# s-elkazdadi/ddp-pinocchio

Measured on AMD Instinct MI355X. Metric: DDP iterations/sec (fwd+bwd sweep), Talos nq=38 T=200, higher is better.
Workload: dtype f64

## Files before the change

ddp_pinocchio_amd/csrc/lin_static.hip:

```cpp
#include <float.h>
#include <math.h>
#include <stdlib.h>

#include <type_traits>
#include <utility>

#include "internal.h"
#include "lin_common.h"
#include "rbd.h"

#ifndef DEV_NO_EMIT
#define DEV_NO_EMIT 0
#endif
namespace {

struct TopoTalos38 {
  static constexpr int N = 38;
  static constexpr int parent[N] = {-1, 0, 1, 2, 3, 4,
                                    5, 6, 7, 8, 9, 10,
                                    5, 12, 13, 14, 15, 16,
                                    5, 18,
                                    19, 20, 21, 22, 23, 24, 25, 26,
                                    19, 28, 29, 30, 31, 32, 33, 34,
                                    19, 36};
  static constexpr int prismatic[N] = {1, 1, 1, 0, 0, 0, 0, 0, 0, 0, 0, 0, 0, 0, 0, 0, 0, 0, 0,
                                       0, 0, 0, 0, 0, 0, 0, 0, 0, 0, 0, 0, 0, 0, 0, 0, 0, 0, 0};
};

struct TopoChain6 {
  static constexpr int N = 6;
  static constexpr int parent[N] = {-1, 0, 1, 2, 3, 4};
  static constexpr int prismatic[N] = {0, 0, 0, 0, 0, 0};
};

}
#include "topo_extra.h"
namespace {

template <class T> constexpr bool has_child(int k) {
  for (int c = k + 1; c < T::N; ++c) if (T::parent[c] == k) return true;
  return false;
}
template <class T> constexpr int largest_child(int k) {
  int r = -1;
  for (int c = k + 1; c < T::N; ++c) if (T::parent[c] == k) r = c;
  return r;
}
template <class T> constexpr bool first_contrib(int k) { return T::parent[k] >= 0 && largest_child<T>(T::parent[k]) == k; }

template <class T>
bool topo_matches(const DevModel& m) {
  if (m.kind != DDP_HIP_MODEL_TREE || m.nv != T::N) return false;
  for (int i = 0; i < T::N; ++i)
    if (m.parent[i] != T::parent[i] || (m.jtype[i] == DDP_HIP_JOINT_PRISMATIC) != (T::prismatic[i] != 0)) return false;
  return true;
}

template <class T>
struct TauState {
  double acc[T::N][6];
  double uu[T::N];
};

template <class T, int K, int QS>
__device__ __forceinline__ void tau_up(const DevModel& m, const double* __restrict__ qc, const double* __restrict__ vc,
                                       double tauK, TauState<T>& s) {
  constexpr int o = T::prismatic[K] ? 3 : 0;
  const double* E = qc + K * QS;
  const double* r = E + 9;
  const double* U = E + 12;
  const double dinv = E[18];
  const double* pA0 = vc + K * rbd::VC_STRIDE + 6;
  const double* Iac = vc + K * rbd::VC_STRIDE + 12;
  const double* a = m.axis[K];
  double pAi[6];
  if constexpr (has_child<T>(K)) {
#pragma unroll
    for (int k = 0; k < 6; ++k) pAi[k] = s.acc[K][k];
  } else {
#pragma unroll
    for (int k = 0; k < 6; ++k) pAi[k] = pA0[k];
  }
  double sp = 0;
#pragma unroll
  for (int k = 0; k < 3; ++k) sp += a[k] * pAi[o + k];
  const double ui = tauK - sp;
  s.uu[K] = ui;
  constexpr int par = T::parent[K];
  if constexpr (par >= 0) {
    double pa[6], fp[6];
#pragma unroll
    for (int k = 0; k < 6; ++k) pa[k] = pAi[k] + Iac[k] + U[k] * (ui * dinv);
    rbd::xform_force_T(E, r, pa, fp);
    if constexpr (first_contrib<T>(K)) {
      const double* pp0 = vc + par * rbd::VC_STRIDE + 6;
#pragma unroll
      for (int k = 0; k < 6; ++k) s.acc[par][k] = pp0[k] + fp[k];
    } else {
#pragma unroll
      for (int k = 0; k < 6; ++k) s.acc[par][k] += fp[k];
    }
  }
  if constexpr (QS == rbd::QC_STRIDE || (K % 2) == 0) __builtin_amdgcn_sched_barrier(0);
}

template <class T, int K, int QS>
__device__ __forceinline__ void tau_down(const DevModel& m, const double* __restrict__ qc, const double* __restrict__ vc,
                                         TauState<T>& s) {
  constexpr int o = T::prismatic[K] ? 3 : 0;
  const double* E = qc + K * QS;
  const double* r = E + 9;
  const double* U = E + 12;
  const double dinv = E[18];
  const double* cb = vc + K * rbd::VC_STRIDE;
  double ap[6];
  constexpr int par = T::parent[K];
  if constexpr (par >= 0) rbd::xform_motion(E, r, s.acc[par], ap);
  else {
    const double a0[6] = {0, 0, 0, -m.gravity[0], -m.gravity[1], -m.gravity[2]};
    rbd::xform_motion(E, r, a0, ap);
  }
  double sum = 0;
#pragma unroll
  for (int k = 0; k < 6; ++k) { ap[k] += cb[k]; sum += U[k] * ap[k]; }
  const double qd = (s.uu[K] - sum) * dinv;
  s.uu[K] = qd;
  if constexpr (has_child<T>(K)) {
    const double* a = m.axis[K];
#pragma unroll
    for (int k = 0; k < 6; ++k) s.acc[K][k] = ap[k];
    s.acc[K][o] += a[0] * qd; s.acc[K][o + 1] += a[1] * qd; s.acc[K][o + 2] += a[2] * qd;
  }
  if constexpr (QS == rbd::QC_STRIDE || (K % 2) == 0) __builtin_amdgcn_sched_barrier(0);
}

template <class T, int QS, class TauFn, int... Ks>
__device__ __forceinline__ void tau_up_all(const DevModel& m, const double* __restrict__ qc, const double* __restrict__ vc, TauFn tau,
                                           TauState<T>& s, std::integer_sequence<int, Ks...>) {
  (tau_up<T, T::N - 1 - Ks, QS>(m, qc, vc, tau(T::N - 1 - Ks), s), ...);
}
template <class T, int QS, int HI, class TauFn, int... Ks>
__device__ __forceinline__ void tau_up_range(const DevModel& m, const double* __restrict__ qc, const double* __restrict__ vc, TauFn tau,
                                             TauState<T>& s, std::integer_sequence<int, Ks...>) {
  (tau_up<T, HI - Ks, QS>(m, qc, vc, tau(HI - Ks), s), ...);
}
template <class T, int QS, int... Ks>
__device__ __forceinline__ void tau_down_all(const DevModel& m, const double* __restrict__ qc, const double* __restrict__ vc,
                                             TauState<T>& s, std::integer_sequence<int, Ks...>) {
  (tau_down<T, Ks, QS>(m, qc, vc, s), ...);
}

constexpr int PS = 20;
template <int NV>
__device__ __forceinline__ void stage_placements(double* sp, const double* __restrict__ qc, int lane) {
  for (int idx = lane; idx < NV * 19; idx += LBS) {
    const int K = idx / 19, e = idx - K * 19;
    sp[K * PS + e] = qc[K * rbd::QC_STRIDE + e];
  }
}

template <class T> constexpr bool parents_at_least(int from, int lo) {
  for (int k = from; k < T::N; ++k) if (T::parent[k] < lo) return false;
  return true;
}
template <class T> constexpr int stage_split() {
  for (int kh = T::N / 2; kh > 0; --kh) if (parents_at_least<T>(kh + 1, kh)) return kh;
  return 0;
}

template <int NV, int K0, int K1, bool WITH_V = true>
struct StageRegs {
  static constexpr int NPW = (K1 - K0) * 19, NVW = WITH_V ? (K1 - K0) * rbd::VC_STRIDE : 0;
  static constexpr int CP = (NPW + LBS - 1) / LBS, CV = (NVW + LBS - 1) / LBS;
  double rp[CP], rv[CV > 0 ? CV : 1];
  __device__ __forceinline__ void load(const double* __restrict__ qc, const double* __restrict__ vc, int lane) {
#pragma unroll
    for (int c = 0; c < CP; ++c) {
      int idx = c * LBS + lane;
      idx = idx < NPW ? idx : NPW - 1;
      const int K = K0 + idx / 19, e = idx % 19;
      rp[c] = qc[K * rbd::QC_STRIDE + e];
    }
#pragma unroll
    for (int c = 0; c < CV; ++c) {
      int idx = c * LBS + lane;
      idx = idx < NVW ? idx : NVW - 1;
      rv[c] = vc[K0 * rbd::VC_STRIDE + idx];
    }
  }
  __device__ __forceinline__ void park(double* sp, double* sv, int lane) const {
#pragma unroll
    for (int c = 0; c < CP; ++c) {
      int idx = c * LBS + lane;
      idx = idx < NPW ? idx : NPW - 1;
      const int K = K0 + idx / 19, e = idx % 19;
      sp[K * PS + e] = rp[c];
    }
#pragma unroll
    for (int c = 0; c < CV; ++c) {
      int idx = c * LBS + lane;
      idx = idx < NVW ? idx : NVW - 1;
      sv[K0 * rbd::VC_STRIDE + idx] = rv[c];
    }
  }
};

__device__ __forceinline__ void tri_index(int64_t q, int Wd, int& ii, int& jj) {
  int a = (int)floor(((2.0 * Wd - 1.0) - sqrt((2.0 * Wd - 1.0) * (2.0 * Wd - 1.0) - 8.0 * (double)q)) * 0.5);
  if (a < 0) a = 0;
  while ((int64_t)a * (2 * Wd - a - 1) / 2 > q) --a;
  while ((int64_t)(a + 1) * (2 * Wd - a - 2) / 2 <= q) ++a;
  ii = a;
  jj = (int)(q - (int64_t)a * (2 * Wd - a - 1) / 2) + a + 1;
}

template <int NV, int NP = LBS>
struct OutStage {
  double qdd[NP * (NV + 1)];
  int pij[NP];
};

template <int NV, int NP>
__device__ __forceinline__ void offdiag_emit(const LinParams& p, OutStage<NV, NP>& S, bool valid, int i, int j, int64_t bt,
                                             const double* __restrict__ xg, double dt, int pass = 0) {
  constexpr int n = 2 * NV, mm = NV;
  constexpr int RW = 16, NJ = (n + RW - 1) / RW, GRP = LBS / RW, PPG = NP / GRP, NB = NP == LBS ? 2 : 1;
  static_assert(PPG % NB == 0, "points per group");
  const double eps = sqrt(sqrt(DBL_EPSILON));
  const double eps2 = eps * eps;
  const int lane = threadIdx.x;
  if (lane / NP == pass) S.pij[lane % NP] = i | (j << 8) | ((valid ? 1 : 0) << 16);
  double* const fxx = p.fxx + bt * n * n * n;
  double* const fux = p.fux + bt * n * mm * n;
  double* const fuu = p.fuu + bt * n * mm * mm;
  const double* const fxb = p.fx + bt * n * n;
  const double* const fub = p.fu + bt * n * mm;
  __syncthreads();
  const int kk = lane % RW, grp = lane / RW;
  const double* f0 = p.f_val + bt * n;
  double f0k[NJ], xk[NJ], xvk[NJ];
#pragma unroll
  for (int jx = 0; jx < NJ; ++jx) {
    const int k = kk + RW * jx;
    const int kc = k < n ? k : n - 1;
    f0k[jx] = f0[kc];
    xk[jx] = xg[kc];
    xvk[jx] = kc < NV ? xg[NV + kc] : 0.0;
  }
  if (DEV_NO_EMIT) return;
  for (int pt = 0; pt < PPG; pt += NB) {
    double a1[NB][NJ], a2[NB][NJ], d1[NB][NJ], d2[NB][NJ];
    double* o0[NB];
    double* o1[NB];
    int ie[NB], je[NB], ee[NB];
#pragma unroll
    for (int u = 0; u < NB; ++u) {
      const int e = (pt + u) * GRP + grp;
      ee[u] = e;
      const int pk = S.pij[e];
      const int i1 = pk & 255, j1 = (pk >> 8) & 255;
      ie[u] = i1;
      je[u] = j1;
      const bool at_x_1 = i1 < n, at_x_2 = j1 < n;
      const int idx_1 = at_x_1 ? i1 : i1 - n, idx_2 = at_x_2 ? j1 : j1 - n;
      double* tensor;
      int L;
      if (at_x_1) { if (at_x_2) { tensor = fxx; L = n; } else { tensor = fux; L = mm; } }
      else { tensor = fuu; L = mm; }
      o0[u] = (pk >> 16) ? tensor + (int64_t)idx_2 * n + (int64_t)idx_1 * n * L : nullptr;
      o1[u] = ((pk >> 16) && at_x_1 == at_x_2 && !p.skip_qv_mirror) ? tensor + (int64_t)idx_1 * n + (int64_t)idx_2 * n * L : nullptr;
      if (o0[u]) {
        const double* q0 = at_x_1 ? fxb + (int64_t)idx_1 * n : fub + (int64_t)idx_1 * n;
        const double* q1 = at_x_2 ? fxb + (int64_t)idx_2 * n : fub + (int64_t)idx_2 * n;
        const double* q2 = at_x_1 ? fxx + (int64_t)idx_1 * n + (int64_t)idx_1 * n * n : fuu + (int64_t)idx_1 * n + (int64_t)idx_1 * n * mm;
        const double* q3 = at_x_2 ? fxx + (int64_t)idx_2 * n + (int64_t)idx_2 * n * n : fuu + (int64_t)idx_2 * n + (int64_t)idx_2 * n * mm;
#pragma unroll
        for (int jx = 0; jx < NJ; ++jx) {
          const int k = kk + RW * jx;
          const int kc = k < n ? k : n - 1;
          a1[u][jx] = q0[kc]; a2[u][jx] = q1[kc]; d1[u][jx] = q2[kc]; d2[u][jx] = q3[kc];
        }
      }
    }
#pragma unroll
    for (int u = 0; u < NB; ++u) {
      if (!o0[u]) continue;
#pragma unroll
      for (int jx = 0; jx < NJ; ++jx) {
        const int k = kk + RW * jx;
        if (k >= n) continue;
        if (p.skip_top && k < NV && !((ie[u] < n && ie[u] % NV == k) || (je[u] < n && je[u] % NV == k))) continue;
        double xs = k == ie[u] ? xk[jx] + eps : xk[jx];
        if (k == je[u]) xs = xs + eps;
        double fv;
        if (k < NV) {
          double xv = (NV + k) == ie[u] ? xvk[jx] + eps : xvk[jx];
          if (NV + k == je[u]) xv = xv + eps;
          const double vo = dt * xv;
          fv = xs + vo;
        } else {
          fv = xs + S.qdd[ee[u] * (NV + 1) + (k - NV)] * dt;
        }
        double df = fv - f0k[jx];
        df -= eps * a1[u][jx];
        df -= eps * a2[u][jx];
        df *= 2;
        const double val = 0.5 * (df / eps2 - d1[u][jx] - d2[u][jx]);
        o0[u][k] = val;
        if (o1[u]) o1[u][k] = val;
      }
    }
  }
}

template <int NV>
struct RowStage {
  double q[(NV + 2) * (NV + 1)];
};

template <int NV, bool DIAG_ROW, class ST>
__device__ __forceinline__ void rowblock_emit(const ST& S, int lane, int i, int jb, double* __restrict__ out, double* __restrict__ mirror,
                                              int64_t mstride, const double* __restrict__ a2, const double* __restrict__ d2, int64_t dstride,
                                              double dt, const double* __restrict__ f0g, const double* __restrict__ a1g,
                                              double* __restrict__ d1g, const double* __restrict__ xg, bool skip_top = false) {
  constexpr int n = 2 * NV, RW = 16, NJ = (n + RW - 1) / RW, CG = LBS / RW, NIT = (NV + CG - 1) / CG;
  const int r1 = i % NV;
  const double eps = sqrt(sqrt(DBL_EPSILON));
  const double eps2 = eps * eps;
  const int kk = lane % RW, cg = lane / RW;
  double xk[NJ], xvk[NJ], f0k[NJ], a1k[NJ], d1k[NJ];
#pragma unroll
  for (int j = 0; j < NJ; ++j) {
    const int k = kk + RW * j;
    const int kc = k < n ? k : n - 1;
    f0k[j] = f0g[kc];
    a1k[j] = a1g[kc];
    double x = xg[kc];
    if (kc == i) x = x + eps;
    xk[j] = x;
    double xv = xg[kc < NV ? NV + kc : kc];
    if (NV + kc == i) xv = xv + eps;
    xvk[j] = xv;
    if constexpr (DIAG_ROW) {
      double fv;
      if (kc < NV) {
        const double vo = dt * xv;
        fv = x + vo;
      } else {
        fv = x + S.q[NV * (NV + 1) + (kc - NV)] * dt;
      }
      double df = fv - f0k[j];
      df -= eps * a1k[j];
      df *= 2;
      const double dd = df / eps2;
      d1k[j] = dd;
      if (cg == 0 && k < n && !(skip_top && k < NV && k != r1)) d1g[k] = dd;
    } else {
      d1k[j] = d1g[kc];
    }
  }
  double va2[2][NJ], vd2[2][NJ];
  auto fetch = [&](int it, double (&A)[NJ], double (&D)[NJ]) {
    const int c = it * CG + cg;
    const int cc = c < NV ? c : NV - 1;
#pragma unroll
    for (int j = 0; j < NJ; ++j) {
      const int k = kk + RW * j;
      const int kc = k < n ? k : n - 1;
      A[j] = a2[kc + cc * n];
      D[j] = d2[kc + cc * dstride];
    }
  };
  auto form = [&](int it, const double (&A)[NJ], const double (&D)[NJ]) {
    const int c = it * CG + cg;
    const bool cv = c < NV;
    const int cc = cv ? c : NV - 1;
    const int jp = jb + cc;
#pragma unroll
    for (int j = 0; j < NJ; ++j) {
      const int k = kk + RW * j;
      if (!(cv && k < n)) continue;
      if (skip_top && k < NV && k != r1 && !(jp < n && jp % NV == k)) continue;
      double x = xk[j];
      if (k == jp) x = x + eps;
      double fv;
      if (k < NV) {
        double xv = xvk[j];
        if (NV + k == jp) xv = xv + eps;
        const double vo = dt * xv;
        fv = x + vo;
      } else {
        fv = x + S.q[cc * (NV + 1) + (k - NV)] * dt;
      }
      double df = fv - f0k[j];
      df -= eps * a1k[j];
      df -= eps * A[j];
      df *= 2;
      const double val = 0.5 * (df / eps2 - d1k[j] - D[j]);
      out[k + c * n] = val;
      if (mirror) mirror[k + c * mstride] = val;
    }
  };
  if (DEV_NO_EMIT) return;
  fetch(0, va2[0], vd2[0]);
  for (int it = 0; it < NIT; it += 2) {
    if (it + 1 < NIT) fetch(it + 1, va2[1], vd2[1]);
    form(it, va2[0], vd2[0]);
    if (it + 1 < NIT) {
      if (it + 2 < NIT) fetch(it + 2, va2[0], vd2[0]);
      form(it + 1, va2[1], vd2[1]);
    }
  }
}

template <class T, bool ROWS>
__global__ __launch_bounds__(LBS, ROWS ? 1 : 3) void lin_static_tau_kernel(LinParams p) {
  constexpr int nv = T::N, n = 2 * nv;
  constexpr int TRI = nv * (nv - 1) / 2, GU = (TRI + LBS - 1) / LBS, G = ROWS ? 2 * nv : GU;
  const int64_t bt = blockIdx.x / G;
  const int g = (int)(blockIdx.x % G) + (ROWS ? 0 : 2 * nv);
  const int lane = threadIdx.x;
  const int64_t Tn = p.d.T;
  const int b = (int)(bt / Tn);
  const int64_t t = bt % Tn;
  const DevModel& m = *p.model;
  int i, j, cfg, vcfg;
  bool valid;
  if (g < nv) { i = g; j = n + lane; cfg = 1 + g; vcfg = nv + 1 + g; valid = lane < nv; }
  else if (g < 2 * nv) { i = g; j = n + lane; cfg = 0; vcfg = 1 + (g - nv); valid = lane < nv; }
  else {
    const int pid = (g - 2 * nv) * LBS + lane;
    valid = pid < TRI;
    tri_index(valid ? pid : 0, nv, i, j);
    i += n; j += n; cfg = 0; vcfg = 0;
  }
  const double eps = sqrt(sqrt(DBL_EPSILON));
  const double* __restrict__ qc = p.qcache + (bt * (nv + 1) + cfg) * (int64_t)nv * rbd::QC_STRIDE;
  const double* __restrict__ vc = p.vcache + (bt * (2 * nv + 1) + vcfg) * (int64_t)nv * rbd::VC_STRIDE;
  const double* __restrict__ xg = p.x + ((int64_t)b * (Tn + 1) + t) * n;
  const double* __restrict__ ug = p.u + ((int64_t)b * Tn + t) * nv;
  const int iu = i - n, ju = j - n;
  __shared__ union TauLds { double P[nv * PS + nv * rbd::VC_STRIDE]; RowStage<nv> S; OutStage<nv, LBS / 2> O; } s_lds;
  double* s_P = s_lds.P;
  double* s_V = s_P + nv * PS;
  constexpr int KH = stage_split<T>();
  StageRegs<nv, 0, (KH > 0) ? KH : 1> lower;
  {
    StageRegs<nv, KH, nv> upper;
    upper.load(qc, vc, lane);
    lower.load(qc, vc, lane);
    upper.park(s_P, s_V, lane);
    rbd::coop_sync<true>();
  }
  TauState<T> s;
  auto tau = [&](int k) { double v = ug[k]; if (k == iu) v = v + eps; if (k == ju) v = v + eps; return v; };
  static_assert(parents_at_least<T>(KH + 1, KH), "the first half of the pass must not reach below record KH");
  tau_up_range<T, PS, nv - 1>(m, s_P, s_V, tau, s, std::make_integer_sequence<int, nv - 1 - KH>{});
  lower.park(s_P, s_V, lane);
  rbd::coop_sync<true>();
  tau_up_range<T, PS, KH>(m, s_P, s_V, tau, s, std::make_integer_sequence<int, KH + 1>{});
  tau_down_all<T, PS>(m, s_P, s_V, s, std::make_integer_sequence<int, nv>{});
  __builtin_amdgcn_sched_barrier(0);
  typedef __attribute__((address_space(4))) const LinParams* kernarg_t;
  const kernarg_t kp = (kernarg_t)__builtin_amdgcn_kernarg_segment_ptr();
  if constexpr (ROWS) {
    RowStage<nv>& S = s_lds.S;
    const int mm = nv;
    __syncthreads();
    const int row = lane <= nv ? lane : nv + 1;
#pragma unroll
    for (int k = 0; k < nv; ++k) S.q[row * (nv + 1) + k] = s.uu[k];
    __syncthreads();
    rowblock_emit<nv, true>(S, lane, i, n, kp->fux + bt * n * mm * n + (int64_t)i * n * mm, nullptr, 0, kp->fu + bt * n * mm,
                            kp->fuu + bt * n * mm * mm, (int64_t)n + (int64_t)n * mm, m.dt, kp->f_val + bt * n,
                            kp->fx + bt * n * n + (int64_t)i * n, kp->fxx + bt * n * n * n + (int64_t)i * n + (int64_t)i * n * n, xg, kp->skip_top != 0);
  } else {
    OutStage<nv, LBS / 2>& S = s_lds.O;
    LinParams po;
    po.f_val = kp->f_val; po.fx = kp->fx; po.fu = kp->fu; po.fxx = kp->fxx; po.fux = kp->fux; po.fuu = kp->fuu; po.skip_qv_mirror = kp->skip_qv_mirror; po.skip_top = kp->skip_top;
    const double dt = m.dt;
    __syncthreads();
#pragma unroll 1
    for (int pass = 0; pass < 2; ++pass) {
      if (pass) __syncthreads();
      if (lane / (LBS / 2) == pass) {
#pragma unroll
        for (int k = 0; k < nv; ++k) S.qdd[(lane % (LBS / 2)) * (nv + 1) + k] = s.uu[k];
      }
      offdiag_emit<nv, LBS / 2>(po, S, valid, i, j, bt, xg, dt, pass);
    }
  }
}

template <class T> constexpr int n_children(int k) {
  int c = 0;
  for (int j = k + 1; j < T::N; ++j) if (T::parent[j] == k) ++c;
  return c;
}
template <class T> constexpr bool chain_start(int k) { return T::parent[k] < 0 || T::parent[k] != k - 1 || n_children<T>(T::parent[k]) > 1; }
template <class T> constexpr bool chain_end(int k) { return k == T::N - 1 || chain_start<T>(k + 1); }
template <class T> constexpr int chain_first(int k) { while (!chain_start<T>(k)) --k; return k; }
template <class T> constexpr int max_chain() {
  int best = 1;
  for (int k = 0; k < T::N; ++k)
    if (chain_end<T>(k)) { const int len = k - chain_first<T>(k) + 1; if (len > best) best = len; }
  return best;
}

template <class T>
struct VelState {
  double vel[T::N][6];
  double acc[T::N][6];
  double uu[T::N];
};

template <int UQS_, int QS_ = rbd::QC_STRIDE>
struct VelCtx {
  static constexpr int UQS = UQS_;
  static constexpr int QS = QS_;
  const DevModel* m;
  const double* qp;
  const double* __restrict__ qc;
  const double* __restrict__ xg;
  const double* __restrict__ ug;
  double* uq;
  int i, j;
  double eps;
  template <int K> __device__ __forceinline__ const double* er(double*) const { return qp + K * QS; }
  template <int K> __device__ __forceinline__ const double* er_down(double* b) const { return er<K>(b); }
  template <int K> __device__ __forceinline__ const double* ud() const { return qp + K * QS + 12; }
  template <int K> __device__ __forceinline__ void ia_cb(const double*, const double* cb, double* Iac) const { rbd::sym6_mv(qc + K * rbd::QC_STRIDE + 19, cb, Iac); }
  template <int K> __device__ __forceinline__ const double* ud_down() const { return ud<K>(); }
};

template <int NV, class C>
__device__ __forceinline__ double lane_v(const C& c, int K) {
  double v = c.xg[NV + K];
  if (NV + K == c.i) v = v + c.eps;
  if (NV + K == c.j) v = v + c.eps;
  return v;
}

template <class T, int K, class C>
__device__ __forceinline__ void joint_vel(const C& c, const double* vel_par, double* vel) {
  constexpr int o = T::prismatic[K] ? 3 : 0;
  double Pb[12];
  const double* E = c.template er<K>(Pb);
  const double* r = E + 9;
  const double* a = c.m->axis[K];
  const double vK = lane_v<T::N>(c, K);
  double vJ[6] = {0, 0, 0, 0, 0, 0};
  vJ[o] = a[0] * vK; vJ[o + 1] = a[1] * vK; vJ[o + 2] = a[2] * vK;
  if constexpr (T::parent[K] >= 0) rbd::xform_motion(E, r, vel_par, vel);
  else {
#pragma unroll
    for (int k = 0; k < 6; ++k) vel[k] = 0.0;
  }
#pragma unroll
  for (int k = 0; k < 6; ++k) vel[k] += vJ[k];
}
template <class T, int K, class C>
__device__ __forceinline__ void vel_from_root(const C& c, double* vel) {
  if constexpr (T::parent[K] >= 0) {
    double vp[6];
    vel_from_root<T, T::parent[K]>(c, vp);
    joint_vel<T, K>(c, vp, vel);
  } else {
    joint_vel<T, K>(c, nullptr, vel);
  }
}
template <class T, int K, class C>
__device__ __forceinline__ void bias_force0(const C& c, const double* vel, double* pA) {
  double Iv[6];
  rbd::sym6_mv(c.m->I6[K], vel, Iv);
  rbd::crf(vel, Iv, pA);
}

template <class T, int K, int E, class C>
__device__ __forceinline__ void chain_down(const C& c, VelState<T>& s) {
  if constexpr (T::parent[K] >= 0) joint_vel<T, K>(c, s.vel[T::parent[K]], s.vel[K]);
  else joint_vel<T, K>(c, nullptr, s.vel[K]);
  __builtin_amdgcn_sched_barrier(0);
  if constexpr (K < E) chain_down<T, K + 1, E>(c, s);
}

template <class T, int K, int F, class C>
__device__ __forceinline__ void chain_up(const C& c, VelState<T>& s) {
  constexpr int o = T::prismatic[K] ? 3 : 0;
  double Pb[12];
  const double* E = c.template er<K>(Pb);
  const double* r = E + 9;
  const double* U = c.template ud<K>();
  const double dinv = U[6];
  const double* a = c.m->axis[K];
  double pAi[6];
  if constexpr (has_child<T>(K)) {
#pragma unroll
    for (int k = 0; k < 6; ++k) pAi[k] = s.acc[K][k];
  } else {
    bias_force0<T, K>(c, s.vel[K], pAi);
  }
  double sp = 0;
#pragma unroll
  for (int k = 0; k < 3; ++k) sp += a[k] * pAi[o + k];
  const double ui = c.ug[K] - sp;
  if constexpr (C::UQS == 0) s.uu[K] = ui; else c.uq[K * C::UQS] = ui;
  constexpr int par = T::parent[K];
  if constexpr (par >= 0) {
    const double vK = lane_v<T::N>(c, K);
    double vJ[6] = {0, 0, 0, 0, 0, 0}, cb[6], pa[6], Iac[6], fp[6];
    vJ[o] = a[0] * vK; vJ[o + 1] = a[1] * vK; vJ[o + 2] = a[2] * vK;
    rbd::crm(s.vel[K], vJ, cb);
    c.template ia_cb<K>(U, cb, Iac);
#pragma unroll
    for (int k = 0; k < 6; ++k) pa[k] = pAi[k] + Iac[k] + U[k] * (ui * dinv);
    rbd::xform_force_T(E, r, pa, fp);
    if constexpr (first_contrib<T>(K)) {
      double p0[6];
      bias_force0<T, par>(c, s.vel[par], p0);
#pragma unroll
      for (int k = 0; k < 6; ++k) s.acc[par][k] = p0[k] + fp[k];
    } else {
#pragma unroll
      for (int k = 0; k < 6; ++k) s.acc[par][k] += fp[k];
    }
  }
  __builtin_amdgcn_sched_barrier(0);
  if constexpr (K > F) chain_up<T, K - 1, F>(c, s);
}

template <class T, int K, class C>
__device__ __forceinline__ void chain_at(const C& c, VelState<T>& s) {
  if constexpr (chain_end<T>(K)) {
    constexpr int F = chain_first<T>(K), P = T::parent[F];
    if constexpr (P >= 0) {
      if constexpr (first_contrib<T>(F) && n_children<T>(P) > 1) vel_from_root<T, P>(c, s.vel[P]);
    }
    chain_down<T, F, K>(c, s);
    chain_up<T, K, F>(c, s);
  }
}
template <class T, class C, int... Ks>
__device__ __forceinline__ void vel_up_all(const C& c, VelState<T>& s, std::integer_sequence<int, Ks...>) {
  (chain_at<T, T::N - 1 - Ks>(c, s), ...);
}

template <class T, int K, class C>
__device__ __forceinline__ void vel_down(const C& c, VelState<T>& s) {
  constexpr int o = T::prismatic[K] ? 3 : 0;
  constexpr int par = T::parent[K];
  double Pb[12];
  const double* E = c.template er_down<K>(Pb);
  const double* r = E + 9;
  const double* U = c.template ud_down<K>();
  const double dinv = U[6];
  const double* a = c.m->axis[K];
  const double vK = lane_v<T::N>(c, K);
  double vJ[6] = {0, 0, 0, 0, 0, 0}, vel[6], cb[6], ap[6];
  vJ[o] = a[0] * vK; vJ[o + 1] = a[1] * vK; vJ[o + 2] = a[2] * vK;
  if constexpr (par >= 0) {
    rbd::xform_motion(E, r, s.vel[par], vel);
    rbd::xform_motion(E, r, s.acc[par], ap);
  } else {
    const double a0[6] = {0, 0, 0, -c.m->gravity[0], -c.m->gravity[1], -c.m->gravity[2]};
#pragma unroll
    for (int k = 0; k < 6; ++k) vel[k] = 0.0;
    rbd::xform_motion(E, r, a0, ap);
  }
#pragma unroll
  for (int k = 0; k < 6; ++k) vel[k] += vJ[k];
  rbd::crm(vel, vJ, cb);
  double sum = 0;
#pragma unroll
  for (int k = 0; k < 6; ++k) { ap[k] += cb[k]; sum += U[k] * ap[k]; }
  double ui;
  if constexpr (C::UQS == 0) ui = s.uu[K]; else ui = c.uq[K * C::UQS];
  const double qd = (ui - sum) * dinv;
  if constexpr (C::UQS == 0) s.uu[K] = qd; else c.uq[K * C::UQS] = qd;
  if constexpr (has_child<T>(K)) {
#pragma unroll
    for (int k = 0; k < 6; ++k) { s.vel[K][k] = vel[k]; s.acc[K][k] = ap[k]; }
    s.acc[K][o] += a[0] * qd; s.acc[K][o + 1] += a[1] * qd; s.acc[K][o + 2] += a[2] * qd;
  }
  __builtin_amdgcn_sched_barrier(0);
}
template <class T, class C, int... Ks>
__device__ __forceinline__ void vel_down_all(const C& c, VelState<T>& s, std::integer_sequence<int, Ks...>) {
  (vel_down<T, Ks>(c, s), ...);
}

template <class T, bool ROWS>
__global__ __launch_bounds__(LBS, ROWS ? 3 : 2) void lin_static_vel_kernel(LinParams p) {
  constexpr int nv = T::N, n = 2 * nv;
  constexpr int TRI = nv * (nv - 1) / 2, GU = (TRI + LBS - 1) / LBS, G = ROWS ? nv : GU;
  const int64_t bt = blockIdx.x / G;
  const int g = (int)(blockIdx.x % G);
  const int lane = threadIdx.x;
  const int64_t Tn = p.d.T;
  const int b = (int)(bt / Tn);
  const int64_t t = bt % Tn;
  int i, j, cfg;
  bool valid;
  if (ROWS) { i = g; j = nv + lane; cfg = 1 + g; valid = lane < nv; }
  else {
    const int pid = g * LBS + lane;
    valid = pid < TRI;
    tri_index(valid ? pid : 0, nv, i, j);
    i += nv; j += nv; cfg = 0;
  }
  struct PairStage { OutStage<nv, LBS / 2> O; double spare[nv + 1]; };
  using Stage = typename std::conditional<ROWS, RowStage<nv>, PairStage>::type;
  __shared__ union VelLds { Stage S; double P[nv * rbd::QC_STRIDE]; } s_lds;
  Stage& S = s_lds.S;
  double* s_P = s_lds.P;
  VelCtx<0, rbd::QC_STRIDE> c;
  c.m = p.model;
  c.qc = p.qcache + (bt * (nv + 1) + cfg) * (int64_t)nv * rbd::QC_STRIDE;
  c.qp = s_P;
  c.xg = p.x + ((int64_t)b * (Tn + 1) + t) * n;
  c.ug = p.u + ((int64_t)b * Tn + t) * nv;
  c.i = i; c.j = j;
  c.eps = sqrt(sqrt(DBL_EPSILON));
  c.uq = nullptr;
  {
    constexpr int NW = nv * rbd::QC_STRIDE, CW = (NW + LBS - 1) / LBS;
    double rq[CW];
#pragma unroll
    for (int r = 0; r < CW; ++r) { const int idx = r * LBS + lane; rq[r] = c.qc[idx < NW ? idx : NW - 1]; }
#pragma unroll
    for (int r = 0; r < CW; ++r) { const int idx = r * LBS + lane; s_P[idx < NW ? idx : NW - 1] = rq[r]; }
    c.qc = s_P;
    rbd::coop_sync<true>();
  }
  VelState<T> s;
  vel_up_all<T>(c, s, std::make_integer_sequence<int, nv>{});
  vel_down_all<T>(c, s, std::make_integer_sequence<int, nv>{});
  __builtin_amdgcn_sched_barrier(0);
  typedef __attribute__((address_space(4))) const LinParams* kernarg_t;
  const kernarg_t kp = (kernarg_t)__builtin_amdgcn_kernarg_segment_ptr();
  const double dt = c.m->dt;
  if constexpr (ROWS) {
    double* fxx = kp->fxx + bt * n * n * n;
    const double* fxb = kp->fx + bt * n * n;
    __syncthreads();
    const int row = valid ? lane : nv;
#pragma unroll
    for (int k = 0; k < nv; ++k) S.q[row * (nv + 1) + k] = s.uu[k];
    __syncthreads();
    rowblock_emit<nv, false>(S, lane, i, nv, fxx + (int64_t)nv * n + (int64_t)i * n * n,
                             kp->skip_qv_mirror ? nullptr : fxx + (int64_t)i * n + (int64_t)nv * n * n, (int64_t)n * n,
                             fxb + (int64_t)nv * n, fxx + (int64_t)nv * n + (int64_t)nv * n * n, (int64_t)n + (int64_t)n * n, dt,
                             kp->f_val + bt * n, fxb + (int64_t)i * n, fxx + (int64_t)i * n + (int64_t)i * n * n, c.xg, kp->skip_top != 0);
  } else {
    constexpr int NP = LBS / 2;
    LinParams po;
    po.f_val = kp->f_val; po.fx = kp->fx; po.fu = kp->fu; po.fxx = kp->fxx; po.fux = kp->fux; po.fuu = kp->fuu; po.skip_qv_mirror = kp->skip_qv_mirror; po.skip_top = kp->skip_top;
    __syncthreads();
    double* const own = &S.O.qdd[(lane % NP) * (nv + 1)];
    double* const row = lane < NP ? own : S.spare;
#pragma unroll
    for (int k = 0; k < nv; ++k) row[k] = s.uu[k];
#pragma unroll 1
    for (int pass = 0; pass < 2; ++pass) {
      if (pass) {
        __syncthreads();
        if (lane >= NP) {
#pragma unroll
          for (int k = 0; k < nv; ++k) own[k] = s.uu[k];
        }
      }
      offdiag_emit<nv, NP>(po, S.O, valid, i, j, bt, c.xg, dt, pass);
    }
  }
}

constexpr int WS_PER_JOINT = 8;

template <class T>
// ... 593 lines not shown
  if constexpr (!DIAG) {
    if (double* ao = kp->accel_out) {
      ao += bt * (3 * nv + 1) * nv;
      double* al = ao + (LEVEL - 1) * nv * nv;
      for (int e = lane; e < nv * nv; e += LBS) { const int c = e / nv; al[e] = s_q[c * (nv + 1) + (e - c * nv)]; }
      if (LEVEL == 2 && lane < nv) ao[3 * nv * nv + lane] = s_q[nv * (nv + 1) + lane];
      return;
    }
  }
  double* fcol = LEVEL == 3 ? kp->fu + bt * n * nv : kp->fx + bt * n * n + (LEVEL == 2 ? nv * n : 0);
  double* out = fcol;
  int64_t ostride = n;
  if constexpr (DIAG) {
    if (LEVEL == 3) { out = kp->fuu + bt * n * nv * nv; ostride = n + (int64_t)n * nv; }
    else { ostride = n + (int64_t)n * n; out = kp->fxx + bt * n * n * n + (LEVEL == 2 ? nv * ostride : 0); }
  }
  first_output<nv, DIAG>(s_q, lane, LEVEL == 1 ? 0 : (LEVEL == 2 ? nv : n), out, ostride, fcol, kp->f_val + bt * n, xg, model->dt, eps, kp->skip_top != 0);
}

template <class T, int K>
__device__ __forceinline__ void placement_static(const DevModel& m, double q, double* P) {
  const double* Rp = m.Rp[K];
  const double* a = m.axis[K];
  double* E = P;
  double* r = P + 9;
  if constexpr (!T::prismatic[K]) {
    double sn, cs;
    sincos(q, &sn, &cs);
    const double Kx[9] = {0, -a[2], a[1], a[2], 0, -a[0], -a[1], a[0], 0};
    double K2[9], RJ[9], Rc[9];
    rbd::mm3(Kx, Kx, K2);
    const double omc = 1.0 - cs;
#pragma unroll
    for (int k = 0; k < 9; ++k) RJ[k] = sn * Kx[k] + omc * K2[k];
    RJ[0] += 1.0; RJ[4] += 1.0; RJ[8] += 1.0;
    rbd::mm3(Rp, RJ, Rc);
#pragma unroll
    for (int k = 0; k < 3; ++k)
#pragma unroll
      for (int l = 0; l < 3; ++l) E[3 * k + l] = Rc[3 * l + k];
    r[0] = m.pp[K][0]; r[1] = m.pp[K][1]; r[2] = m.pp[K][2];
  } else {
    const double dd[3] = {a[0] * q, a[1] * q, a[2] * q};
    double Rd[3];
    rbd::mv3(Rp, dd, Rd);
#pragma unroll
    for (int k = 0; k < 3; ++k)
#pragma unroll
      for (int l = 0; l < 3; ++l) E[3 * k + l] = Rp[3 * l + k];
    r[0] = m.pp[K][0] + Rd[0]; r[1] = m.pp[K][1] + Rd[1]; r[2] = m.pp[K][2] + Rd[2];
  }
}

struct QvCtx {
  const DevModel* __restrict__ m;
  const double* __restrict__ xg;
  double* __restrict__ qc;
  double* __restrict__ vc;
  double* lvel;
  int jn;
  double eps;
};
template <class T>
struct QvState {
  double vel[T::N][6];
  double accI[T::N][21];
};
template <class T, int K>
__device__ __forceinline__ void qv_placement(const QvCtx& c, double* P) {
  double q = c.xg[K];
  if (K == c.jn) q = q + c.eps;
  placement_static<T, K>(*c.m, q, P);
}
template <class T, int K>
__device__ __forceinline__ void qv_joint_vel(const QvCtx& c, const double* P, const double* vel_par, double* vel) {
  constexpr int o = T::prismatic[K] ? 3 : 0;
  const double* a = c.m->axis[K];
  const double vK = c.xg[T::N + K];
  double vJ[6] = {0, 0, 0, 0, 0, 0};
  vJ[o] = a[0] * vK; vJ[o + 1] = a[1] * vK; vJ[o + 2] = a[2] * vK;
  if constexpr (T::parent[K] >= 0) rbd::xform_motion(P, P + 9, vel_par, vel);
  else {
#pragma unroll
    for (int k = 0; k < 6; ++k) vel[k] = 0.0;
  }
#pragma unroll
  for (int k = 0; k < 6; ++k) vel[k] += vJ[k];
}
template <class T, int K>
__device__ __forceinline__ void qv_vel_from_root(const QvCtx& c, double* vel) {
  double P[12];
  qv_placement<T, K>(c, P);
  if constexpr (T::parent[K] >= 0) {
    double vp[6];
    qv_vel_from_root<T, T::parent[K]>(c, vp);
    qv_joint_vel<T, K>(c, P, vp, vel);
  } else {
    qv_joint_vel<T, K>(c, P, nullptr, vel);
  }
}
template <class T, int K, int F, int E>
__device__ __forceinline__ void qv_chain_down(const QvCtx& c, double* cur) {
  double P[12], vel[6];
  qv_placement<T, K>(c, P);
  if constexpr (T::parent[K] >= 0) qv_joint_vel<T, K>(c, P, cur, vel);
  else qv_joint_vel<T, K>(c, P, nullptr, vel);
#pragma unroll
  for (int k = 0; k < 6; ++k) { cur[k] = vel[k]; c.lvel[((K - F) * 6 + k) * LBS] = vel[k]; }
  __builtin_amdgcn_sched_barrier(0);
  if constexpr (K < E) qv_chain_down<T, K + 1, F, E>(c, cur);
}
template <class T, int K, int F>
__device__ __forceinline__ void qv_chain_up(const QvCtx& c, QvState<T>& s) {
  constexpr int o = T::prismatic[K] ? 3 : 0;
  const double* a = c.m->axis[K];
  double P[12], IA[21], U[6], Ia[21], vel[6];
  qv_placement<T, K>(c, P);
#pragma unroll
  for (int k = 0; k < 6; ++k) vel[k] = c.lvel[((K - F) * 6 + k) * LBS];
  if constexpr (has_child<T>(K)) {
#pragma unroll
    for (int k = 0; k < 21; ++k) IA[k] = s.accI[K][k];
  } else {
#pragma unroll
    for (int k = 0; k < 21; ++k) IA[k] = c.m->I6[K][k];
  }
  double d = 0;
#pragma unroll
  for (int r = 0; r < 6; ++r) U[r] = IA[rbd::sidx(r, o)] * a[0] + IA[rbd::sidx(r, o + 1)] * a[1] + IA[rbd::sidx(r, o + 2)] * a[2];
#pragma unroll
  for (int k = 0; k < 3; ++k) d += a[k] * U[o + k];
  const double dinv = 1.0 / d;
#pragma unroll
  for (int r = 0; r < 6; ++r)
#pragma unroll
    for (int cc = 0; cc <= r; ++cc) Ia[rbd::sidx(r, cc)] = IA[rbd::sidx(r, cc)] - U[r] * U[cc] * dinv;
  constexpr int par = T::parent[K];
  if constexpr (par >= 0) {
    if constexpr (first_contrib<T>(K)) {
#pragma unroll
      for (int k = 0; k < 21; ++k) s.accI[par][k] = c.m->I6[par][k];
    }
    rbd::add_xtix(P, P + 9, Ia, s.accI[par]);
  }
  const double vK = c.xg[T::N + K];
  double vJ[6] = {0, 0, 0, 0, 0, 0}, cb[6], pA[6], Iv[6], Iac[6];
  vJ[o] = a[0] * vK; vJ[o + 1] = a[1] * vK; vJ[o + 2] = a[2] * vK;
  rbd::crm(vel, vJ, cb);
  rbd::sym6_mv(c.m->I6[K], vel, Iv);
  rbd::crf(vel, Iv, pA);
  rbd::sym6_mv(Ia, cb, Iac);
  double* qo = c.qc + K * rbd::QC_STRIDE;
#pragma unroll
  for (int k = 0; k < 12; ++k) qo[k] = P[k];
#pragma unroll
  for (int k = 0; k < 6; ++k) qo[12 + k] = U[k];
  qo[18] = dinv;
#pragma unroll
  for (int k = 0; k < 21; ++k) qo[19 + k] = Ia[k];
  double* vo = c.vc + K * rbd::VC_STRIDE;
#pragma unroll
  for (int k = 0; k < 6; ++k) { vo[k] = cb[k]; vo[6 + k] = pA[k]; vo[12 + k] = Iac[k]; }
  __builtin_amdgcn_sched_barrier(0);
  if constexpr (K > F) qv_chain_up<T, K - 1, F>(c, s);
}
template <class T, int K>
__device__ __forceinline__ void qv_chain_at(const QvCtx& c, QvState<T>& s) {
  if constexpr (chain_end<T>(K)) {
    constexpr int F = chain_first<T>(K), P = T::parent[F];
    double cur[6] = {0, 0, 0, 0, 0, 0};
    if constexpr (P >= 0) {
      if constexpr (first_contrib<T>(F) && n_children<T>(P) > 1) qv_vel_from_root<T, P>(c, s.vel[P]);
#pragma unroll
      for (int k = 0; k < 6; ++k) cur[k] = s.vel[P][k];
    }
    qv_chain_down<T, F, F, K>(c, cur);
    qv_chain_up<T, K, F>(c, s);
  }
}
template <class T, int... Ks>
__device__ __forceinline__ void qv_all(const QvCtx& c, QvState<T>& s, std::integer_sequence<int, Ks...>) {
  (qv_chain_at<T, T::N - 1 - Ks>(c, s), ...);
}

template <class T>
__global__ __launch_bounds__(LBS, 2) void lin_static_qvcache_kernel(LinParams p, const DevModel* __restrict__ model, const double* __restrict__ xs,
                                                                 double* __restrict__ qcache, double* __restrict__ vcache) {
  constexpr int nv = T::N, n = 2 * nv, MAXCH = max_chain<T>();
  const int lane = threadIdx.x;
  const int64_t Tn = p.d.T;
  const int64_t e = (int64_t)blockIdx.x * LBS + lane;
  const int64_t bt = e / p.ncfg;
  const int cfgi = (int)(e - bt * p.ncfg);
  const int b = (int)(bt / Tn);
  const int64_t t = bt % Tn;
  __shared__ double s_vel[MAXCH * 6 * LBS];
  if (bt >= p.d.batch * Tn) return;
  QvCtx c;
  c.m = model;
  c.xg = xs + ((int64_t)b * (Tn + 1) + t) * n;
  c.qc = qcache + (bt * p.ncfg + cfgi) * (int64_t)nv * rbd::QC_STRIDE;
  c.vc = vcache + (bt * p.nvcfg + (cfgi == 0 ? 0 : nv + cfgi)) * (int64_t)nv * rbd::VC_STRIDE;
  c.lvel = s_vel + lane;
  c.jn = cfgi - 1;
  c.eps = sqrt(sqrt(DBL_EPSILON));
  QvState<T> s;
  qv_all<T>(c, s, std::make_integer_sequence<int, nv>{});
}

template <class T, int K>
__device__ __forceinline__ void vc_joint(const DevModel& m, const double* __restrict__ qc, const double* __restrict__ xg, int iv, double eps,
                                         double (&vel)[T::N][6], double* __restrict__ vc) {
  constexpr int o = T::prismatic[K] ? 3 : 0;
  const double* E = qc + K * rbd::QC_STRIDE;
  const double* r = E + 9;
  const double* Ia = E + 19;
  const double* a = m.axis[K];
  double vK = xg[T::N + K];
  if (K == iv) vK = vK + eps;
  double vJ[6] = {0, 0, 0, 0, 0, 0}, v[6], cb[6], pA[6], Iv[6], Iac[6];
  vJ[o] = a[0] * vK; vJ[o + 1] = a[1] * vK; vJ[o + 2] = a[2] * vK;
  if constexpr (T::parent[K] >= 0) rbd::xform_motion(E, r, vel[T::parent[K]], v);
  else {
#pragma unroll
    for (int k = 0; k < 6; ++k) v[k] = 0.0;
  }
#pragma unroll
  for (int k = 0; k < 6; ++k) { v[k] += vJ[k]; vel[K][k] = v[k]; }
  rbd::crm(v, vJ, cb);
  rbd::sym6_mv(m.I6[K], v, Iv);
  rbd::crf(v, Iv, pA);
  rbd::sym6_mv(Ia, cb, Iac);
  double* vo = vc + K * rbd::VC_STRIDE;
#pragma unroll
  for (int k = 0; k < 6; ++k) { vo[k] = cb[k]; vo[6 + k] = pA[k]; vo[12 + k] = Iac[k]; }
  __builtin_amdgcn_sched_barrier(0);
}
template <class T, int... Ks>
__device__ __forceinline__ void vc_all(const DevModel& m, const double* __restrict__ qc, const double* __restrict__ xg, int iv, double eps,
                                       double (&vel)[T::N][6], double* __restrict__ vc, std::integer_sequence<int, Ks...>) {
  (vc_joint<T, Ks>(m, qc, xg, iv, eps, vel, vc), ...);
}
template <class T>
__global__ __launch_bounds__(LBS) void lin_static_vcache_kernel(LinParams p, const DevModel* __restrict__ model, const double* __restrict__ xs,
                                                                const double* __restrict__ qcache, double* __restrict__ vcache) {
  constexpr int nv = T::N, n = 2 * nv;
  const int64_t bt = blockIdx.x;
  const int lane = threadIdx.x;
  const int64_t Tn = p.d.T;
  const int b = (int)(bt / Tn);
  const int64_t t = bt % Tn;
  if (lane >= nv) return;
  const double* __restrict__ qc = qcache + (bt * (nv + 1)) * (int64_t)nv * rbd::QC_STRIDE;
  const double* __restrict__ xg = xs + ((int64_t)b * (Tn + 1) + t) * n;
  double* __restrict__ vc = vcache + (bt * (2 * nv + 1) + 1 + lane) * (int64_t)nv * rbd::VC_STRIDE;
  double vel[nv][6];
  vc_all<T>(*model, qc, xg, lane, sqrt(sqrt(DBL_EPSILON)), vel, vc, std::make_integer_sequence<int, nv>{});
}

}

int lin_static_supported(const DevModel& m) {
  if (m.ff) return 0;
  if (topo_matches<TopoTalos38>(m)) return 1;
  if (topo_matches<TopoChain6>(m)) return 2;
#define DDP_TOPO_MATCH(ID, TOPO) if (topo_matches<TOPO>(m)) return (ID) - 1;
  DDP_TOPO_EXTRA(DDP_TOPO_MATCH)
#undef DDP_TOPO_MATCH
  return 0;
}

int64_t lin_static_ws_per_bt(const DevModel& m) {
  const int64_t nv = m.nv, TRI = nv * (nv - 1) / 2, GU = (TRI + LBS - 1) / LBS;
  int64_t rec = 0;
  for (int i = 0; i < nv; ++i)
    for (int j = i + 1; j < nv; ++j) {
      const auto anc = [&](int a, int x) { for (int k = m.parent[x]; k >= 0; k = m.parent[k]) if (k == a) return true; return false; };
      int a = m.parent[i];
      while (a >= 0 && !anc(a, j)) a = m.parent[a];
      for (; a >= 0; a = m.parent[a]) ++rec;
    }
  const int64_t sweep = GU * nv * WS_PER_JOINT * LBS, splice = rec * SREC;
  return sweep > splice ? sweep : splice;
}

template <class T>
static void launch_first_columns(ddp_hip_ctx* ctx, const LinParams& p, bool with_u) {
  const int64_t BT = ctx->d.batch * ctx->d.T;
  constexpr int nv = T::N, TRI = nv * (nv - 1) / 2, GU = (TRI + LBS - 1) / LBS;
  const int64_t per = ctx->lin_qws_bt * GU;
  for (int64_t bt0 = 0; bt0 < BT; bt0 += per) {
    const int64_t nb = BT - bt0 < per ? BT - bt0 : per;
    hipLaunchKernelGGL((lin_static_first_kernel<T, 1, false>), dim3((unsigned)nb), dim3(LBS), 0, ctx->stream, p, p.model, p.qcache, p.x, p.u, ctx->lin_qws, bt0);
  }
  hipLaunchKernelGGL((lin_static_first_kernel<T, 2, false>), dim3((unsigned)BT), dim3(LBS), 0, ctx->stream, p, p.model, p.qcache, p.x, p.u, ctx->lin_qws, (int64_t)0);
  if (with_u) hipLaunchKernelGGL((lin_static_first_kernel<T, 3, false>), dim3((unsigned)BT), dim3(LBS), 0, ctx->stream, p, p.model, p.qcache, p.x, p.u, ctx->lin_qws, (int64_t)0);
}

template <class T>
static int lin_static_launch_t(ddp_hip_ctx* ctx, const LinParams& p, StaticLevel level) {
  const int64_t BT = ctx->d.batch * ctx->d.T;
  constexpr int nv = T::N, TRI = nv * (nv - 1) / 2, GU = (TRI + LBS - 1) / LBS;
  if (level == StaticLevel::Torque) {
    hipLaunchKernelGGL((lin_static_tau_kernel<T, true>), dim3((unsigned)(BT * 2 * nv)), dim3(LBS), 0, ctx->stream, p);
    hipLaunchKernelGGL((lin_static_tau_kernel<T, false>), dim3((unsigned)(BT * GU)), dim3(LBS), 0, ctx->stream, p);
  } else if (level == StaticLevel::Caches) {
    hipLaunchKernelGGL((lin_static_qvcache_kernel<T>), dim3((unsigned)((BT * p.ncfg + LBS - 1) / LBS)), dim3(LBS), 0, ctx->stream, p, p.model, p.x, p.qcache, p.vcache);
    if (p.nvcfg > 1) hipLaunchKernelGGL((lin_static_vcache_kernel<T>), dim3((unsigned)BT), dim3(LBS), 0, ctx->stream, p, p.model, p.x, p.qcache, p.vcache);
  } else if (level == StaticLevel::AccelXU || level == StaticLevel::AccelX) {
    if (!p.accel_out) return DDP_HIP_E_ARG;
    hipLaunchKernelGGL((lin_static_qvcache_kernel<T>), dim3((unsigned)((BT * p.ncfg + LBS - 1) / LBS)), dim3(LBS), 0, ctx->stream, p, p.model, p.x, p.qcache, p.vcache);
    launch_first_columns<T>(ctx, p, level == StaticLevel::AccelXU);
  } else if (level == StaticLevel::FirstOrder) {
    launch_first_columns<T>(ctx, p, true);
  } else if (level == StaticLevel::UDiagonal) {
    hipLaunchKernelGGL((lin_static_first_kernel<T, 3, true>), dim3((unsigned)BT), dim3(LBS), 0, ctx->stream, p, p.model, p.qcache, p.x, p.u, ctx->lin_qws, (int64_t)0);
  } else if (level == StaticLevel::Configuration && !ctx->sw.cfg_full_aba) {
    constexpr int64_t NREC = spine_records<T>(), SWEEP = (int64_t)GU * nv * WS_PER_JOINT * LBS;
    constexpr int64_t WS_BT = SWEEP > NREC * SREC ? SWEEP : NREC * SREC;
    const int64_t per = NREC > 0 ? ctx->lin_qws_bt * WS_BT / (NREC * SREC) : BT;
    for (int64_t bt0 = 0; bt0 < BT; bt0 += per) {
      const int nb = (int)(BT - bt0 < per ? BT - bt0 : per);
      const dim3 grid((unsigned)((nb + 7) / 8 * 8 * GU));
      hipLaunchKernelGGL((lin_static_spine_kernel<T>), grid, dim3(LBS), 0, ctx->stream, p.model, p.qcache, p.vcache, ctx->lin_qws, bt0, nb);
      hipLaunchKernelGGL((lin_static_cfg_pair_kernel<T>), grid, dim3(LBS), 0, ctx->stream, p, ctx->lin_qws, bt0, nb);
    }
  } else if (level == StaticLevel::Configuration) {
    const int64_t per = ctx->lin_qws_bt;
    hipStream_t s0 = ctx->stream, s1 = ctx->lin_stream2;
    int k = 0;
    for (int64_t bt0 = 0; bt0 < BT; bt0 += per, ++k) {
      const int64_t nb = BT - bt0 < per ? BT - bt0 : per;
      const int w = k & 1;
      double* ws = w ? ctx->lin_qws2 : ctx->lin_qws;
      if (k >= 2) HIP_TRY(hipStreamWaitEvent(s0, ctx->lin_ev_dn[w], 0));
      hipLaunchKernelGGL((lin_static_cfg_up_kernel<T>), dim3((unsigned)(nb * GU)), dim3(LBS), 0, s0, p, p.model, p.qcache, p.x, p.u, ws, bt0);
      HIP_TRY(hipEventRecord(ctx->lin_ev_up[w], s0));
      HIP_TRY(hipStreamWaitEvent(s1, ctx->lin_ev_up[w], 0));
      hipLaunchKernelGGL((lin_static_cfg_down_kernel<T>), dim3((unsigned)(nb * GU)), dim3(LBS), 0, s1, p, p.model, p.qcache, p.x, p.u, ws, bt0);
      HIP_TRY(hipEventRecord(ctx->lin_ev_dn[w], s1));
    }
    if (k >= 1) HIP_TRY(hipStreamWaitEvent(s0, ctx->lin_ev_dn[0], 0));
    if (k >= 2) HIP_TRY(hipStreamWaitEvent(s0, ctx->lin_ev_dn[1], 0));
  } else if (level == StaticLevel::Velocity) {
    hipLaunchKernelGGL((lin_static_vel_kernel<T, true>), dim3((unsigned)(BT * nv)), dim3(LBS), 0, ctx->stream, p);
    hipLaunchKernelGGL((lin_static_vel_kernel<T, false>), dim3((unsigned)(BT * GU)), dim3(LBS), 0, ctx->stream, p);
  }
  HIP_TRY(hipGetLastError());
  return DDP_HIP_OK;
}

int lin_static_launch(ddp_hip_ctx* ctx, const LinParams& p, StaticLevel level) {
  if (ctx->plan.topo == 1) return lin_static_launch_t<TopoTalos38>(ctx, p, level);
  if (ctx->plan.topo == 2) return lin_static_launch_t<TopoChain6>(ctx, p, level);
#define DDP_TOPO_LAUNCH(ID, TOPO) if (ctx->plan.topo == (ID) - 1) return lin_static_launch_t<TOPO>(ctx, p, level);
  DDP_TOPO_EXTRA(DDP_TOPO_LAUNCH)
#undef DDP_TOPO_LAUNCH
  return DDP_HIP_E_UNSUPPORTED;
}
```

Before: 704.7.

## Pack several velocity-row torque sweeps per workgroup with per-slot LDS velocity blocks

Splits the torque-linearisation row kernel into a configuration-row launch and a new velocity-row launch. The velocity-row launch packs several rows (nv+1 lanes each) into one workgroup, possibly two wavefronts wide. Each slot has its own bank-staggered LDS velocity-cache block, so lanes that previously sat idle beyond nv are used and fewer blocks are launched. In exchange it adds a serial per-row emit loop with extra barriers, larger LDS use, and a third kernel launch.

```diff
diff --git a/ddp_pinocchio_amd/csrc/lin_static.hip b/ddp_pinocchio_amd/csrc/lin_static.hip
--- a/ddp_pinocchio_amd/csrc/lin_static.hip
+++ b/ddp_pinocchio_amd/csrc/lin_static.hip
@@ -168,39 +168,47 @@
   return 0;
 }
 
-template <int NV, int K0, int K1, bool WITH_V = true>
+template <int NV, int K0, int K1, bool WITH_V = true, int NT = LBS, int R = 1, int VB = NV * rbd::VC_STRIDE>
 struct StageRegs {
-  static constexpr int NPW = (K1 - K0) * 19, NVW = WITH_V ? (K1 - K0) * rbd::VC_STRIDE : 0;
-  static constexpr int CP = (NPW + LBS - 1) / LBS, CV = (NVW + LBS - 1) / LBS;
+  static constexpr int NPW = (K1 - K0) * 19, NV1 = (K1 - K0) * rbd::VC_STRIDE, NVW = WITH_V ? R * NV1 : 0;
+  static constexpr int CP = (NPW + NT - 1) / NT, CV = (NVW + NT - 1) / NT;
   double rp[CP], rv[CV > 0 ? CV : 1];
-  __device__ __forceinline__ void load(const double* __restrict__ qc, const double* __restrict__ vc, int lane) {
+  __device__ __forceinline__ void load(const double* __restrict__ qc, const double* __restrict__ vc, int lane, int nrows = 1) {
 #pragma unroll
     for (int c = 0; c < CP; ++c) {
-      int idx = c * LBS + lane;
+      int idx = c * NT + lane;
       idx = idx < NPW ? idx : NPW - 1;
       const int K = K0 + idx / 19, e = idx % 19;
       rp[c] = qc[K * rbd::QC_STRIDE + e];
     }
 #pragma unroll
     for (int c = 0; c < CV; ++c) {
-      int idx = c * LBS + lane;
+      int idx = c * NT + lane;
       idx = idx < NVW ? idx : NVW - 1;
-      rv[c] = vc[K0 * rbd::VC_STRIDE + idx];
+      if constexpr (R == 1) rv[c] = vc[K0 * rbd::VC_STRIDE + idx];
+      else {
+        const int r = idx / NV1, e = idx - r * NV1;
+        rv[c] = vc[(r < nrows ? r : nrows - 1) * (NV * rbd::VC_STRIDE) + K0 * rbd::VC_STRIDE + e];
+      }
     }
   }
   __device__ __forceinline__ void park(double* sp, double* sv, int lane) const {
 #pragma unroll
     for (int c = 0; c < CP; ++c) {
-      int idx = c * LBS + lane;
+      int idx = c * NT + lane;
       idx = idx < NPW ? idx : NPW - 1;
       const int K = K0 + idx / 19, e = idx % 19;
       sp[K * PS + e] = rp[c];
     }
 #pragma unroll
     for (int c = 0; c < CV; ++c) {
-      int idx = c * LBS + lane;
+      int idx = c * NT + lane;
       idx = idx < NVW ? idx : NVW - 1;
-      sv[K0 * rbd::VC_STRIDE + idx] = rv[c];
+      if constexpr (R == 1) sv[K0 * rbd::VC_STRIDE + idx] = rv[c];
+      else {
+        const int r = idx / NV1, e = idx - r * NV1;
+        sv[r * VB + K0 * rbd::VC_STRIDE + e] = rv[c];
+      }
     }
   }
 };
@@ -318,12 +326,12 @@
   double q[(NV + 2) * (NV + 1)];
 };
 
-template <int NV, bool DIAG_ROW, class ST>
+template <int NV, bool DIAG_ROW, int NT = LBS, class ST>
 __device__ __forceinline__ void rowblock_emit(const ST& S, int lane, int i, int jb, double* __restrict__ out, double* __restrict__ mirror,
                                               int64_t mstride, const double* __restrict__ a2, const double* __restrict__ d2, int64_t dstride,
                                               double dt, const double* __restrict__ f0g, const double* __restrict__ a1g,
                                               double* __restrict__ d1g, const double* __restrict__ xg, bool skip_top = false) {
-  constexpr int n = 2 * NV, RW = 16, NJ = (n + RW - 1) / RW, CG = LBS / RW, NIT = (NV + CG - 1) / CG;
+  constexpr int n = 2 * NV, RW = 16, NJ = (n + RW - 1) / RW, CG = NT / RW, NIT = (NV + CG - 1) / CG;
   const int r1 = i % NV;
   const double eps = sqrt(sqrt(DBL_EPSILON));
   const double eps2 = eps * eps;
@@ -413,23 +421,60 @@
   }
 }
 
-template <class T, bool ROWS>
-__global__ __launch_bounds__(LBS, ROWS ? 1 : 3) void lin_static_tau_kernel(LinParams p) {
-  constexpr int nv = T::N, n = 2 * nv;
-  constexpr int TRI = nv * (nv - 1) / 2, GU = (TRI + LBS - 1) / LBS, G = ROWS ? 2 * nv : GU;
+template <int P>
+struct RowGroup {
+  static constexpr int W = 2 * P <= LBS ? 1 : 2, R = W * LBS / P, NT = W * LBS;
+};
+template <int NV, int R> constexpr int vblock_stride() {
+  int vb = NV * rbd::VC_STRIDE + (NV * rbd::VC_STRIDE) % 2;
+  for (;; vb += 2) {
+    bool ok = true;
+    for (int sd = 1; sd < R; ++sd) { const int d = (sd * vb) % 32; if (d < 2 || d > 30) ok = false; }
+    if (ok) return vb;
+  }
+}
+template <int W> __device__ __forceinline__ void group_sync() {
+  if constexpr (W == 1) rbd::coop_sync<true>();
+  else {
+    __builtin_amdgcn_fence(__ATOMIC_RELEASE, "workgroup", "local");
+    __builtin_amdgcn_s_barrier();
+    __builtin_amdgcn_fence(__ATOMIC_ACQUIRE, "workgroup", "local");
+  }
+}
+
+enum : int { TAU_PAIRS = 0, TAU_QROWS = 1, TAU_VROWS = 2 };
+template <class T, int MODE>
+struct TauShape {
+  using RG = RowGroup<T::N + 1>;
+  static constexpr int P = T::N + 1;
+  static constexpr int W = MODE == TAU_VROWS ? RG::W : 1, R = MODE == TAU_VROWS ? RG::R : 1, NT = W * LBS;
+  static constexpr int NG = (T::N + R - 1) / R;
+  static constexpr int VB = vblock_stride<T::N, R>();
+};
+
+template <class T, int MODE>
+__global__ __launch_bounds__((TauShape<T, MODE>::NT), (MODE == TAU_QROWS ? 1 : 3)) void lin_static_tau_kernel(LinParams p) {
+  using SH = TauShape<T, MODE>;
+  constexpr int nv = T::N, n = 2 * nv, P = SH::P, W = SH::W, R = SH::R, NT = SH::NT, VB = SH::VB;
+  constexpr int TRI = nv * (nv - 1) / 2, GU = (TRI + LBS - 1) / LBS, G = MODE == TAU_PAIRS ? GU : MODE == TAU_QROWS ? nv : SH::NG;
   const int64_t bt = blockIdx.x / G;
-  const int g = (int)(blockIdx.x % G) + (ROWS ? 0 : 2 * nv);
+  const int g = (int)(blockIdx.x % G);
   const int lane = threadIdx.x;
   const int64_t Tn = p.d.T;
   const int b = (int)(bt / Tn);
   const int64_t t = bt % Tn;
   const DevModel& m = *p.model;
-  int i, j, cfg, vcfg;
+  int i, j, cfg, vcfg, nrows = 1, slot = 0, pt = lane;
   bool valid;
-  if (g < nv) { i = g; j = n + lane; cfg = 1 + g; vcfg = nv + 1 + g; valid = lane < nv; }
-  else if (g < 2 * nv) { i = g; j = n + lane; cfg = 0; vcfg = 1 + (g - nv); valid = lane < nv; }
-  else {
-    const int pid = (g - 2 * nv) * LBS + lane;
+  if constexpr (MODE == TAU_QROWS) { i = g; j = n + lane; cfg = 1 + g; vcfg = nv + 1 + g; valid = lane < nv; }
+  else if constexpr (MODE == TAU_VROWS) {
+    const int row0 = g * R;
+    nrows = nv - row0 < R ? nv - row0 : R;
+    slot = lane / P; pt = lane - slot * P;
+    i = nv + row0;
+    j = n + pt; cfg = 0; vcfg = 1 + row0; valid = slot < nrows && pt < nv;
+  } else {
+    const int pid = g * LBS + lane;
     valid = pid < TRI;
     tri_index(valid ? pid : 0, nv, i, j);
     i += n; j += n; cfg = 0; vcfg = 0;
@@ -440,30 +485,31 @@
   const double* __restrict__ xg = p.x + ((int64_t)b * (Tn + 1) + t) * n;
   const double* __restrict__ ug = p.u + ((int64_t)b * Tn + t) * nv;
   const int iu = i - n, ju = j - n;
-  __shared__ union TauLds { double P[nv * PS + nv * rbd::VC_STRIDE]; RowStage<nv> S; OutStage<nv, LBS / 2> O; } s_lds;
+  __shared__ union TauLds { double P[nv * PS + (R - 1) * VB + nv * rbd::VC_STRIDE]; RowStage<nv> S; OutStage<nv, LBS / 2> O; } s_lds;
   double* s_P = s_lds.P;
   double* s_V = s_P + nv * PS;
+  const double* s_Vl = s_V + (slot < R ? slot : R - 1) * VB;
   constexpr int KH = stage_split<T>();
-  StageRegs<nv, 0, (KH > 0) ? KH : 1> lower;
+  StageRegs<nv, 0, (KH > 0) ? KH : 1, true, NT, R, VB> lower;
   {
-    StageRegs<nv, KH, nv> upper;
-    upper.load(qc, vc, lane);
-    lower.load(qc, vc, lane);
+    StageRegs<nv, KH, nv, true, NT, R, VB> upper;
+    upper.load(qc, vc, lane, nrows);
+    lower.load(qc, vc, lane, nrows);
     upper.park(s_P, s_V, lane);
-    rbd::coop_sync<true>();
+    group_sync<W>();
   }
   TauState<T> s;
   auto tau = [&](int k) { double v = ug[k]; if (k == iu) v = v + eps; if (k == ju) v = v + eps; return v; };
   static_assert(parents_at_least<T>(KH + 1, KH), "the first half of the pass must not reach below record KH");
-  tau_up_range<T, PS, nv - 1>(m, s_P, s_V, tau, s, std::make_integer_sequence<int, nv - 1 - KH>{});
+  tau_up_range<T, PS, nv - 1>(m, s_P, s_Vl, tau, s, std::make_integer_sequence<int, nv - 1 - KH>{});
   lower.park(s_P, s_V, lane);
-  rbd::coop_sync<true>();
-  tau_up_range<T, PS, KH>(m, s_P, s_V, tau, s, std::make_integer_sequence<int, KH + 1>{});
-  tau_down_all<T, PS>(m, s_P, s_V, s, std::make_integer_sequence<int, nv>{});
+  group_sync<W>();
+  tau_up_range<T, PS, KH>(m, s_P, s_Vl, tau, s, std::make_integer_sequence<int, KH + 1>{});
+  tau_down_all<T, PS>(m, s_P, s_Vl, s, std::make_integer_sequence<int, nv>{});
   __builtin_amdgcn_sched_barrier(0);
   typedef __attribute__((address_space(4))) const LinParams* kernarg_t;
   const kernarg_t kp = (kernarg_t)__builtin_amdgcn_kernarg_segment_ptr();
-  if constexpr (ROWS) {
+  if constexpr (MODE == TAU_QROWS) {
     RowStage<nv>& S = s_lds.S;
     const int mm = nv;
     __syncthreads();
@@ -474,6 +520,23 @@
     rowblock_emit<nv, true>(S, lane, i, n, kp->fux + bt * n * mm * n + (int64_t)i * n * mm, nullptr, 0, kp->fu + bt * n * mm,
                             kp->fuu + bt * n * mm * mm, (int64_t)n + (int64_t)n * mm, m.dt, kp->f_val + bt * n,
                             kp->fx + bt * n * n + (int64_t)i * n, kp->fxx + bt * n * n * n + (int64_t)i * n + (int64_t)i * n * n, xg, kp->skip_top != 0);
+  } else if constexpr (MODE == TAU_VROWS) {
+    RowStage<nv>& S = s_lds.S;
+    const int mm = nv;
+    const double dt = m.dt;
+#pragma unroll 1
+    for (int r = 0; r < nrows; ++r) {
+      group_sync<W>();
+      if (slot == r) {
+#pragma unroll
+        for (int k = 0; k < nv; ++k) S.q[pt * (nv + 1) + k] = s.uu[k];
+      }
+      group_sync<W>();
+      const int ir = i + r;
+      rowblock_emit<nv, true, NT>(S, lane, ir, n, kp->fux + bt * n * mm * n + (int64_t)ir * n * mm, nullptr, 0, kp->fu + bt * n * mm,
+                                  kp->fuu + bt * n * mm * mm, (int64_t)n + (int64_t)n * mm, dt, kp->f_val + bt * n,
+                                  kp->fx + bt * n * n + (int64_t)ir * n, kp->fxx + bt * n * n * n + (int64_t)ir * n + (int64_t)ir * n * n, xg, kp->skip_top != 0);
+    }
   } else {
     OutStage<nv, LBS / 2>& S = s_lds.O;
     LinParams po;
@@ -1673,8 +1736,10 @@
   const int64_t BT = ctx->d.batch * ctx->d.T;
   constexpr int nv = T::N, TRI = nv * (nv - 1) / 2, GU = (TRI + LBS - 1) / LBS;
   if (level == StaticLevel::Torque) {
-    hipLaunchKernelGGL((lin_static_tau_kernel<T, true>), dim3((unsigned)(BT * 2 * nv)), dim3(LBS), 0, ctx->stream, p);
-    hipLaunchKernelGGL((lin_static_tau_kernel<T, false>), dim3((unsigned)(BT * GU)), dim3(LBS), 0, ctx->stream, p);
+    using VR = TauShape<T, TAU_VROWS>;
+    hipLaunchKernelGGL((lin_static_tau_kernel<T, TAU_QROWS>), dim3((unsigned)(BT * nv)), dim3(LBS), 0, ctx->stream, p);
+    hipLaunchKernelGGL((lin_static_tau_kernel<T, TAU_VROWS>), dim3((unsigned)(BT * VR::NG)), dim3(VR::NT), 0, ctx->stream, p);
+    hipLaunchKernelGGL((lin_static_tau_kernel<T, TAU_PAIRS>), dim3((unsigned)(BT * GU)), dim3(LBS), 0, ctx->stream, p);
   } else if (level == StaticLevel::Caches) {
     hipLaunchKernelGGL((lin_static_qvcache_kernel<T>), dim3((unsigned)((BT * p.ncfg + LBS - 1) / LBS)), dim3(LBS), 0, ctx->stream, p, p.model, p.x, p.qcache, p.vcache);
     if (p.nvcfg > 1) hipLaunchKernelGGL((lin_static_vcache_kernel<T>), dim3((unsigned)BT), dim3(LBS), 0, ctx->stream, p, p.model, p.x, p.qcache, p.vcache);
```

Result: slower. 695.8 (-1.3%).
